# LDeakin/VkVolume

Measured on AMD Instinct MI355X. Metric: Mray/s, higher is better.
Workload: dtype f32

## Files before the change

### vkvolume_amd/csrc/raymarch.hip

```cpp
#include <algorithm>
#include <cmath>
#include <cstdio>
#include <cstdlib>
#include <cstring>
#include <mutex>
#include <new>
#include <vector>

#include "raymarch_inst.hpp"
#include "launchers.hpp"

constexpr int kCostBins = 1024;

__device__ __forceinline__ void tile_order_from_cost(uint32_t *__restrict__ cost, uint32_t *__restrict__ order_out, uint32_t count)
{
	__shared__ uint32_t s_bin[kCostBins];
	constexpr int       kPerThread = 40;
	for (int b = threadIdx.x; b < kCostBins; b += blockDim.x)
		s_bin[b] = 0;
	__syncthreads();
	for (uint32_t base = 0; base < count; base += 256u * kPerThread)
	{
		uint32_t c[kPerThread];
#pragma unroll
// ... 248 lines not shown
{
	const uint32_t tiles_x = (iw + tw - 1) / tw, tiles_y = (ih + th - 1) / th;
	*out = VkvTileRect{0u, 0u, tiles_x, tiles_y};
	double    b[4];
	const int kind = screen_bound(rc->camera_pos_tex, rg->dir00, rg->ddx, rg->ddy, rc->plane_tex, b);
	if (kind == kScreenBoundNone)
		return;
	if (kind == kScreenBoundEmpty || b[0] >= (double) iw || b[2] >= (double) ih)
	{
		*out = VkvTileRect{0u, 0u, 1u, 1u};
		return;
	}
	const uint32_t x0 = b[0] <= 0.0 ? 0u : (uint32_t) b[0], y0 = b[2] <= 0.0 ? 0u : (uint32_t) b[2];
	const uint32_t x1 = b[1] >= (double) (iw - 1) ? iw - 1 : (uint32_t) b[1], y1 = b[3] >= (double) (ih - 1) ? ih - 1 : (uint32_t) b[3];
	const uint32_t q = align > 1 ? align : 1u;
	uint32_t       tx0 = (x0 / tw) / q * q, ty0 = (y0 / th) / q * q;
	uint32_t       tx1 = std::min(tiles_x, (x1 / tw + q) / q * q), ty1 = std::min(tiles_y, (y1 / th + q) / q * q);
	*out = VkvTileRect{tx0, ty0, tx1 - tx0, ty1 - ty0};
}

int fill_render_args(vkv_ctx *ctx, const VkvRenderParams *P, const float *alpha_lut, RayMarchArgs &a, hipStream_t s, const VkvTuning &T, bool setup, bool batch)
{
	for (int i = 0; i < 3; ++i)
	{
		a.dir00[i] = P->ray_gen.dir00[i], a.ddx[i] = P->ray_gen.ddx[i], a.ddy[i] = P->ray_gen.ddy[i];
		a.cam[i]        = P->ray_cast.camera_pos_tex[i];
		a.block_size[i] = P->ray_cast.block_size[i];
	}
	for (int i = 0; i < 4; ++i)
		a.plane_tex[i] = P->ray_cast.plane_tex[i];
	for (int i = 0; i < 16; ++i)
		a.model[i] = P->camera.model[i], a.view[i] = P->camera.camera_view[i], a.proj[i] = P->camera.camera_proj[i],
		a.view_proj_inv[i] = P->camera.camera_view_proj_inv[i], a.model_inv[i] = P->camera.model_inv[i];
	a.sampling_factor = P->transfer_function.sampling_factor;
	a.grad_modifier   = P->transfer_function.grad_magnitude_modifier;
	a.W = (int) P->volume_extent.width, a.H = (int) P->volume_extent.height, a.D = (int) P->volume_extent.depth;
	a.mw = (int) P->map_extent.width, a.mh = (int) P->map_extent.height, a.md = (int) P->map_extent.depth;
	a.vol = P->d_volume, a.grad = P->d_gradient, a.tf = P->d_transfer_function;
	a.packed  = static_cast<const uint8_t *>(P->d_packed_volume);
	a.tf_bits = P->d_transfer_function_bits;
	{
		const PackedDims pd = packed_dims(a.W, a.H, a.D);
		a.pmx = pd.mx, a.pmy = pd.my;
	}
	for (int i = 0; i < 8; ++i)
		a.maps[i] = P->d_distance_maps[i];
	a.out_color = P->d_out_color, a.out_rgba8 = P->d_out_rgba8, a.out_counts = P->d_out_counts, a.out_depth = P->d_out_depth;
	a.in_depth         = P->d_in_depth;
	a.depth_attachment = P->options.depth_attachment != 0, a.blend = P->blend_over_target != 0;
	a.img_w = P->image_width, a.img_h = P->image_height;
	a.tile_w = P->tiles.tile_width, a.tile_h = P->tiles.tile_height;
	a.tile_first = P->tiles.tile_first, a.tile_stride = P->tiles.tile_stride, a.tile_count = P->tiles.tile_count, a.compact = P->tiles.compact;
	a.fill_rgba8_rows = (a.out_rgba8 && !a.out_color && !a.out_counts && !a.out_depth && !a.blend && (a.img_w & 3u) == 0 && (((uintptr_t) a.out_rgba8) & 15u) == 0) ? 1u : 0u;
	bool whole_schedule;
	{
		const VkvTileRect &r = P->tiles.rect;
		const uint32_t     full_x = (a.img_w + a.tile_w - 1) / a.tile_w, full_y = (a.img_h + a.tile_h - 1) / a.tile_h;
		bool               whole  = r.w == 0 || r.h == 0;
		a.fill_tiles = 0, a.img_tiles_x = full_x, a.rect_tx0 = a.rect_ty0 = a.rect_th = 0;
		if (!whole && P->tiles.fill_outside)
		{
			if (!batch || T.scheduler == 1 || T.batch_mode == 1 || (uint64_t) full_x * full_y - (uint64_t) r.w * r.h > (uint64_t) kFillPerTile * r.w * r.h)
				whole = true, a.tile_count = full_x * full_y;
			else
				a.fill_tiles = full_x * full_y - r.w * r.h, a.rect_tx0 = r.x0, a.rect_ty0 = r.y0, a.rect_th = r.h;
		}
// ... 126 lines not shown

	const bool ert  = P->options.early_ray_termination != 0;
	const int  grad = !P->transfer_function.use_gradient ? 0 : (P->use_precomputed_gradient ? 1 : 2);
	const bool sort = sched == (int) kSchedLean && ert && apply_feedback(ctx, a, s);
	int        rc2 = launch_single(ctx, P->options.skipping_type, ert, sched, T, grad, a, s);
	if (rc2 == VKV_OK && sort)
	{
		hipLaunchKernelGGL(k_tile_order_from_cost, dim3(1), dim3(256), 0, s, a.tile_cost, a.order_out, a.tile_count);
		rc2 = check_launch(ctx, "render (start order)");
	}
	return rc2;
}

int prepare_render(vkv_ctx *ctx, const VkvRenderParams *P, uint32_t n, hipStream_t s)
{
	const VkvTuning T = tuning_of(ctx);
	float           lut[256] = {};
	for (uint32_t i = 0; i < n; ++i)
	{
		RayMarchArgs a;
		int rc = fill_render_args(ctx, &P[i], lut, a, s, T, true, false);
		if (rc == VKV_OK && P[i].tiles.fill_outside)
			rc = fill_render_args(ctx, &P[i], lut, a, s, T, true, true);
		if (rc != VKV_OK)
			return rc;
		load_render_code(P[i].options.skipping_type, P[i].options.early_ray_termination != 0);
	}
	load_feedback_code();
	if (!stream_scratch(ctx, s, true).p)
		return VKV_E_UNSUPPORTED;
	return VKV_OK;
}

int launch_render_batch(vkv_ctx *ctx, const VkvRenderParams *P, uint32_t n, const float *alpha_luts, hipStream_t s)
{
	static_assert(kMaxBatch * sizeof(RayMarchArgs) <= kScratchBytes - kBatchArgsOffset, "batch argument blocks must fit the stream scratch");
	static_assert(kPullHeadsBytes + kMaxBatch * sizeof(RayMarchArgs) <= kCaptureSlotBytes, "a captured launch's upload must fit its pinned slot");
	static_assert(kPullHeadsBytes + kMaxBatch * sizeof(RayMarchArgs) <= kUploadSlotBytes, "a launch's upload must fit a slot of the block's pinned ring");
	const VkvTuning     T = tuning_of(ctx);
	const StreamScratch scratch = stream_scratch(ctx, s);
	if (!scratch.p)
		return VKV_E_UNSUPPORTED;
	hipStreamCaptureStatus capture = hipStreamCaptureStatusNone;
	const bool             capturing = hipStreamIsCapturing(s, &capture) == hipSuccess && capture == hipStreamCaptureStatusActive;
	const size_t          upload_bytes = kPullHeadsBytes + n * sizeof(RayMarchArgs);
	vkv_ctx::UploadSlot * ring_slot = nullptr;
	for (uint32_t k = 0; k < vkv_ctx::kUploadRing && !capturing && !ring_slot; ++k)
	{
		vkv_ctx::UploadSlot &u = scratch.block->upload[(scratch.block->upload_next + k) % vkv_ctx::kUploadRing];
		if (!u.pinned)
			continue;
		if (u.pending && hipEventQuery(u.done) == hipSuccess)
			u.pending = false;
		if (!u.pending)
		{
			ring_slot                  = &u;
			scratch.block->upload_next = (scratch.block->upload_next + k + 1) % vkv_ctx::kUploadRing;
		}
	}
	(void) hipGetLastError();
	std::vector<uint8_t> pageable;
	if (!ring_slot)
		pageable.resize(upload_bytes);
	uint8_t *const upload = ring_slot ? ring_slot->pinned : pageable.data();
	std::memset(upload, 0, upload_bytes);
	RayMarchArgs *const host = reinterpret_cast<RayMarchArgs *>(upload + kPullHeadsBytes);
	for (uint32_t i = 0; i < n; ++i)
	{
		const int rc = fill_render_args(ctx, &P[i], alpha_luts + (size_t) i * 256, host[i], s, T, false, true);
		if (rc != VKV_OK)
			return rc;
		if (!host[i].packed)
			return set_error(ctx, VKV_E_INVALID_ARGUMENT, "render_batch: frame %u has no packed sampling image (d_packed_volume)", i);
		if (host[i].blocks_per_tile != host[0].blocks_per_tile)
			return set_error(ctx, VKV_E_INVALID_ARGUMENT, "render_batch: frame %u has a different tile size than frame 0", i);
		if (ctx->d_debug_orders && i < ctx->debug_order_frames && ctx->debug_order_count == host[i].tile_count)
			host[i].tile_order = ctx->d_debug_orders + (size_t) i * ctx->debug_order_count;
	}
	uint32_t max_tiles = 0, ref = 0;
	bool     same_count = true;
	for (uint32_t i = n; i-- > 0;)
	{
		max_tiles = std::max(max_tiles, host[i].nblocks ? host[i].tile_count : 0u);
		if (host[i].nblocks)
			ref = i;
	}
	if (max_tiles == 0)
		return VKV_OK;
	for (uint32_t i = 0; i < n; ++i)
		same_count = same_count && host[i].nblocks != 0 && host[i].tile_count == max_tiles;
	bool any_sort = false;
	for (uint32_t i = 0; i < n && P[0].options.early_ray_termination != 0; ++i)
		any_sort = apply_feedback(ctx, host[i], s) || any_sort;
	RayMarchArgs *   d_frames = reinterpret_cast<RayMarchArgs *>(scratch.p + kBatchArgsOffset);
	uint32_t *       d_heads  = reinterpret_cast<uint32_t *>(scratch.p + kBatchArgsOffset - kPullHeadsBytes);
	const void *upload_src = upload;
	struct SlotGuard
	{
		vkv_ctx *ctx;
		size_t   index;
		bool     armed;
		~SlotGuard()
		{
			if (!armed)
				return;
			std::lock_guard<std::mutex> lock(ctx->mutex);
			if (index < ctx->capture_slots.size())
				ctx->capture_slots[index].in_use = false, ctx->capture_slots[index].owner = VkvStreamKey{};
		}
	} slot_guard{ctx, 0, false};
// ... 95 lines not shown
```

### vkvolume_amd/csrc/raymarch_core.hpp

```cpp
#pragma once

#include <type_traits>

#include "vkv_device.hpp"

using namespace vkv;

constexpr int kTraceWords = 10;
constexpr uint32_t kFillPerTile = 3;

struct RayMarchArgs
{
	float dir00[3], ddx[3], ddy[3];
	float cam[3];
	float plane_tex[4];
	float block_size[3];
	float model[16], view[16], proj[16];
	float view_proj_inv[16], model_inv[16];
	float sampling_factor, grad_modifier;
	int W, H, D, mw, mh, md;
	const uint8_t * vol, *grad, *tf;
	const uint8_t * packed;
	int             pmx, pmy;
	const uint32_t *tf_bits;
	const uint8_t * maps[8];
	float *         out_color;
	uint8_t *       out_rgba8;
	uint32_t *      out_counts;
	float *         out_depth;
	const float *   in_depth;
	uint32_t        depth_attachment, blend;
	uint32_t        img_w, img_h, tile_w, tile_h, tiles_x, tile_first, tile_stride, tile_count, compact;
	uint32_t        org_x, org_y;
	uint32_t        fill_tiles, img_tiles_x, rect_tx0, rect_ty0, rect_th;
	uint32_t        fill_rgba8_rows;
	uint32_t        blocks_per_tile_x, blocks_per_tile, nblocks;
	int             test;
	unsigned long long *trace;
	int             back;
	uint32_t        clamp_always;
	float           mapf[3], mapb[3];
	uint32_t        wave_pw_log2;
	const uint32_t *addr_lut;
	uint32_t        lut_y, lut_z, lut_words;
	uint32_t        lut_full;
	uint32_t        cull_x0, cull_x1, cull_y0, cull_y1;
	const uint32_t *tile_order;
	uint32_t        order_h;
	uint32_t *      queue_heads;
	uint32_t *      tile_cost;
	uint32_t *      order_out;
	float           alpha_lut[256];
};

struct Ray
{
	float          ex, ey, ez;
	float          sx, sy, sz;
	float          six, siy, siz;
	const uint8_t *dmap;
	int            n_steps, i, i_min;
	int            ulx, uly, ulz;
	uint32_t       ul;
	int            first_hit;
	bool           occupied;
	float          r, g, b, a;
	float          depth;
	uint32_t       n_vol, n_dist, n_empty;
	uint32_t       o;
	bool           fragment;
};

__device__ __forceinline__ float sample_linear(const uint8_t *__restrict__ tex, int W, int H, int D, float px, float py, float pz)
{
	const float cx = __builtin_fmaf(px, (float) W, -0.5f), cy = __builtin_fmaf(py, (float) H, -0.5f), cz = __builtin_fmaf(pz, (float) D, -0.5f);
	const float fx = __builtin_floorf(cx), fy = __builtin_floorf(cy), fz = __builtin_floorf(cz);
	const float wx = cx - fx, wy = cy - fy, wz = cz - fz;
	const int   ix = (int) fx, iy = (int) fy, iz = (int) fz;
	const int   x0 = i_clamp(ix, 0, W - 1), x1 = i_clamp(ix + 1, 0, W - 1);
	const int   y0 = i_clamp(iy, 0, H - 1), y1 = i_clamp(iy + 1, 0, H - 1);
	const int   z0 = i_clamp(iz, 0, D - 1), z1 = i_clamp(iz + 1, 0, D - 1);
	const size_t r00 = ((size_t) z0 * (size_t) H + (size_t) y0) * (size_t) W, r10 = ((size_t) z0 * (size_t) H + (size_t) y1) * (size_t) W;
	const size_t r01 = ((size_t) z1 * (size_t) H + (size_t) y0) * (size_t) W, r11 = ((size_t) z1 * (size_t) H + (size_t) y1) * (size_t) W;
	const float b000 = tex[r00 + x0], b100 = tex[r00 + x1];
	const float b010 = tex[r10 + x0], b110 = tex[r10 + x1];
	const float b001 = tex[r01 + x0], b101 = tex[r01 + x1];
// ... 648 lines not shown
		}
		if (n_idle == 64)
			break;
		if (active)
		{
			if (ray_event<SKIP, ERT, GRAD, PACKED>(A, R, s_alpha, s_unorm, s_bits, tf_bits))
			{
				ray_finish(A, R, true);
				active = false;
			}
		}
	}
}


struct RmLds
{
	union
	{
		struct
		{
			float    alpha[256];
			uint32_t bits[2048];
			float    unorm[256];
		} g;
		struct
		{
			float  ai[258], ag[258];
			float2 pair[256];
		} s;
	};
};

__device__ __forceinline__ bool tf_is_separable(const RayMarchArgs &A)
{
	return A.tf_bits != nullptr && (A.tf_bits[kTfFlagWord] & kTfFlagSeparable) != 0u;
}

__device__ __forceinline__ bool stage_tables_er(const RayMarchArgs &A, RmLds &L, bool sync = true)
{
	const bool sep = tf_is_separable(A);
	typedef const __attribute__((address_space(1))) uint32_t *global_u32_ptr;
	const global_u32_ptr tf_words = (global_u32_ptr) (uintptr_t) A.tf_bits;
	for (int i = threadIdx.x; i < 256; i += blockDim.x)
	{
		const float a = A.alpha_lut[i];
		if (!sep)
			L.g.alpha[i] = a;
		if (sep)
		{
			const float ai = __uint_as_float(tf_words[kTfAiWord + i]), ag = __uint_as_float(tf_words[kTfAgWord + i]);
			L.s.ai[i] = ai, L.s.ag[i] = ag;
			if (i == 255)
				L.s.ai[256] = ai, L.s.ag[256] = ag;
			L.s.pair[i] = i == 0 ? make_float2(0.0f, 0.0f) : make_float2(a, unorm8(i) * a);
		}
		else
			L.g.unorm[i] = unorm8(i);
	}
	if (!sep && A.tf_bits)
		for (int i = threadIdx.x; i < 2048; i += blockDim.x)
			L.g.bits[i] = A.tf_bits[i];
	if (sync)
		__syncthreads();
	return sep;
}
template <int W>
__device__ __forceinline__ bool block_pixel(const RayMarchArgs &A, uint32_t b, uint32_t rb, uint32_t &px, uint32_t &py, uint32_t &o)
{
	constexpr uint32_t G = 64 / W;
	uint32_t           bx, by;
	const uint32_t     wb = rb / G, g = rb % G;
	if (W == 1)
	{
		const uint32_t pwl = A.wave_pw_log2, pprl = 4u - pwl;
		bx = ((wb & ((1u << pprl) - 1u)) << pwl) + (g & ((1u << pwl) - 1u));
		by = ((wb >> pprl) << (6u - pwl)) + (g >> pwl);
	}
	else
	{
		constexpr uint32_t pw = G >= 32 ? 8 : (G >= 8 ? 4 : 2), ph = G / pw, ppr = 16 / pw;
		bx = (wb % ppr) * pw + g % pw, by = (wb / ppr) * ph + g / pw;
	}
	const uint32_t k = b / A.blocks_per_tile, sb = b % A.blocks_per_tile;
	const uint32_t t  = A.tile_first + k * A.tile_stride;
	const uint32_t lx = (sb % A.blocks_per_tile_x) * 16 + bx, ly = (sb / A.blocks_per_tile_x) * 16 + by;
	px = A.org_x + (t % A.tiles_x) * A.tile_w + lx, py = A.org_y + (t / A.tiles_x) * A.tile_h + ly;
	o  = A.compact ? (k * A.tile_h + ly) * A.tile_w + lx : py * A.img_w + px;
	return px < A.img_w && py < A.img_h;
}
__device__ __forceinline__ int med3_i32(int x, int lo, int hi)
// ... 86 lines not shown
		const float c0 = __builtin_fmaf(wy, c10 - c00, c00), c1 = __builtin_fmaf(wy, c11 - c01, c01);
		out_g = __builtin_fmaf(wz, c1 - c0, c0) * kScale;
	}
}
extern __shared__ __align__(16) uint32_t s_lean_lds[];
static_assert(sizeof(RmLds) % 16 == 0, "the address tables behind RmLds are read as 64-bit words");

typedef __attribute__((address_space(3))) RmLds *   lds_rmlds_ptr;
typedef __attribute__((address_space(3))) uint32_t *lds_u32_ptr;

constexpr uintptr_t kLdsBase = 16;
__device__ __forceinline__ RmLds &lean_lds() { return *(RmLds *) (lds_rmlds_ptr) kLdsBase; }

__device__ __forceinline__ void lean_lds_check()
{
	uint32_t base = (uint32_t) reinterpret_cast<uintptr_t>(s_lean_lds);
	asm volatile("" : "+s"(base));
	if (base != 0u)
		__builtin_trap();
}

__device__ __forceinline__ bool wg_any(bool pred)
{
	uint32_t *flags = (uint32_t *) (lds_u32_ptr) kLdsBase;
	const bool mine = __builtin_amdgcn_ballot_w64(pred) != 0ull;
	if ((threadIdx.x & 63u) == 0u)
		flags[threadIdx.x >> 6] = mine ? 1u : 0u;
	__syncthreads();
	const uint32_t nw  = blockDim.x >> 6;
	const uint4    f   = *reinterpret_cast<const uint4 *>(flags);
	const bool     any = (f.x | (nw > 1u ? f.y : 0u) | (nw > 2u ? f.z : 0u) | (nw > 3u ? f.w : 0u)) != 0u;
	__syncthreads();
	return any;
}

#define s_addr_lut ((uint32_t *) (lds_u32_ptr) (kLdsBase + sizeof(RmLds)))
constexpr uint32_t kLutXm = 96;

__device__ __forceinline__ void stage_addr_lut(const RayMarchArgs &A)
{
	for (uint32_t i = threadIdx.x; i < A.lut_z; i += blockDim.x)
		s_addr_lut[i] = A.addr_lut[i];
	const uint64_t base = reinterpret_cast<uint64_t>(A.packed);
	for (uint32_t i = threadIdx.x; 2 * i + A.lut_z < A.lut_words; i += blockDim.x)
	{
		const uint64_t z = (((uint64_t) A.addr_lut[A.lut_z + 2 * i + 1]) << 32 | A.addr_lut[A.lut_z + 2 * i]) + base;
		s_addr_lut[A.lut_z + 2 * i] = (uint32_t) z, s_addr_lut[A.lut_z + 2 * i + 1] = (uint32_t) (z >> 32);
	}
}

template <bool SC = true>
__device__ __forceinline__ const uint8_t *packed_footprint_lut(const RayMarchArgs &A, float px, float py, float pz, float &wx, float &wy, float &wz)
{
	const float cx = __builtin_fmaf(px, (float) A.W, -0.5f), cy = __builtin_fmaf(py, (float) A.H, -0.5f), cz = __builtin_fmaf(pz, (float) A.D, -0.5f);
	const float fx = __builtin_floorf(cx), fy = __builtin_floorf(cy), fz = __builtin_floorf(cz);
	wx = cx - fx, wy = cy - fy, wz = cz - fz;
	const uint32_t tx = (uint32_t) (SC ? clamp0_i32((int) __builtin_fmaf(fx, 4.0f, 4.0f), 4 * (A.W + 1)) : med3_i32((int) __builtin_fmaf(fx, 4.0f, 4.0f), 0, 4 * (A.W + 1)));
	const uint32_t ty = (uint32_t) (SC ? clamp0_i32((int) __builtin_fmaf(fy, 4.0f, 4.0f), 4 * (A.H + 1)) : med3_i32((int) __builtin_fmaf(fy, 4.0f, 4.0f), 0, 4 * (A.H + 1)));
	const uint32_t tz = (uint32_t) (SC ? clamp0_i32((int) __builtin_fmaf(fz, 4.0f, 4.0f), 4 * (A.D + 1)) : med3_i32((int) __builtin_fmaf(fz, 4.0f, 4.0f), 0, 4 * (A.D + 1)));
	const char *   lut = reinterpret_cast<const char *>(s_addr_lut);
	const uint32_t xi = *reinterpret_cast<const uint32_t *>(lut + (tx & 124u)), xm = *reinterpret_cast<const uint32_t *>(lut + 4u * kLutXm + ((tx >> 5) & ~3u));
	const uint32_t yi = *reinterpret_cast<const uint32_t *>(lut + 128u + (ty & 124u)), ym = *reinterpret_cast<const uint32_t *>(lut + 4u * A.lut_y + ((ty >> 5) & ~3u));
	const uint32_t zi = *reinterpret_cast<const uint32_t *>(lut + 256u + (tz & 124u));
	const uint64_t zm = *reinterpret_cast<const uint64_t *>(lut + 4u * A.lut_z + ((tz >> 4) & ~7u));
	return reinterpret_cast<const uint8_t *>(zm + (((xi + xm) + (yi + ym)) + zi));
}
// ... 28 lines not shown
	uint32_t nvec;
};

__device__ __forceinline__ FullLutCopy full_lut_issue(const RayMarchArgs &A)
{
	typedef const __attribute__((address_space(1))) lut_v4u *global_v4u_ptr;
	FullLutCopy          c;
	const global_v4u_ptr g = (global_v4u_ptr) (uintptr_t) (A.addr_lut + A.lut_full);
	c.nvec                 = ((uint32_t) (A.W + 2 + A.H + 2 + A.D + 2) + 3u) >> 2;
#pragma unroll
	for (uint32_t k = 0; k < kFullCopyRounds; ++k)
		c.r[k] = g[min(threadIdx.x + k * blockDim.x, c.nvec - 1u)];
	return c;
}

__device__ __forceinline__ void full_lut_commit(const RayMarchArgs &A, const FullLutCopy &c, RmLds &L)
{
	static_assert(sizeof(((RmLds *) nullptr)->s) == kFullLutWord * 4, "full tables start behind the separable TF tables");
	typedef const __attribute__((address_space(1))) lut_v4u *global_v4u_ptr;
	lut_v4u *dst = reinterpret_cast<lut_v4u *>(full_lut_base(L));
#pragma unroll
	for (uint32_t k = 0; k < kFullCopyRounds; ++k)
		if (threadIdx.x + k * blockDim.x < c.nvec)
			dst[threadIdx.x + k * blockDim.x] = c.r[k];
	const global_v4u_ptr g = (global_v4u_ptr) (uintptr_t) (A.addr_lut + A.lut_full);
	for (uint32_t i = threadIdx.x + kFullCopyRounds * blockDim.x; i < c.nvec; i += blockDim.x)
		dst[i] = g[i];
}

__device__ __forceinline__ void stage_full_lut(const RayMarchArgs &A, RmLds &L)
{
	const FullLutCopy c = full_lut_issue(A);
	full_lut_commit(A, c, L);
}

struct FullLutConsts
{
	float          w, h, d, oy, oz;
	const uint8_t *base;
};

template <bool SCALAR = false>
__device__ __forceinline__ FullLutConsts full_lut_consts(const RayMarchArgs &A)
{
	FullLutConsts c;
	c.w = (float) A.W, c.h = (float) A.H, c.d = (float) A.D;
	c.base = A.packed;
	c.oy = (float) (4 * (A.W + 2) + 4);
	c.oz = (float) (4 * (A.W + 2 + A.H + 2) + 4);
	if (SCALAR)
		c.w = uniform_f32(c.w), c.h = uniform_f32(c.h), c.d = uniform_f32(c.d), c.oy = uniform_f32(c.oy), c.oz = uniform_f32(c.oz);
	else
		asm volatile("" : "+v"(c.w), "+v"(c.h), "+v"(c.d), "+v"(c.oy), "+v"(c.oz));
	return c;
}

template <bool FREE = false>
__device__ __forceinline__ const uint8_t *packed_footprint_full(const FullLutConsts &C, const RmLds &L, float px, float py, float pz, float &wx, float &wy, float &wz)
{
	const float cx = __builtin_fmaf(px, C.w, -0.5f), cy = __builtin_fmaf(py, C.h, -0.5f), cz = __builtin_fmaf(pz, C.d, -0.5f);
	const float fx = __builtin_floorf(cx), fy = __builtin_floorf(cy), fz = __builtin_floorf(cz);
	wx = cx - fx, wy = cy - fy, wz = cz - fz;
	const int   tx = (int) __builtin_fmaf(FREE ? fx : __builtin_amdgcn_fmed3f(fx, -1.0f, C.w), 4.0f, 4.0f);
	const int   ty = (int) __builtin_fmaf(FREE ? fy : __builtin_amdgcn_fmed3f(fy, -1.0f, C.h), 4.0f, C.oy);
	const int   tz = (int) __builtin_fmaf(FREE ? fz : __builtin_amdgcn_fmed3f(fz, -1.0f, C.d), 4.0f, C.oz);
	const char *   lut = reinterpret_cast<const char *>(full_lut_base(L));
// ... 370 lines not shown
		R.a = R.a > 0.99f ? 1.0f : R.a;
	if (SEP)
		R.r = grey, R.g = grey, R.b = grey;
}

__device__ __forceinline__ uint32_t start_entry(const RayMarchArgs &A, uint32_t r)
{
	const int w = (int) A.tiles_x, h = (int) A.order_h, rings = (min(w, h) + 1) >> 1;
	auto      inner = [&](int j) { return (w - 2 * j > 0 && h - 2 * j > 0) ? (uint32_t) ((w - 2 * j) * (h - 2 * j)) : 0u; };
	const float d = (float) (w - h);
	int         j = (int) (((float) (w + h) - __builtin_sqrtf(d * d + 4.0f * (float) r)) * 0.25f);
	j             = max(0, min(j, rings - 1));
#pragma unroll
	for (int it = 0; it < 2; ++it)
	{
		if (j + 1 < rings && inner(j + 1) > r)
			++j;
		if (j > 0 && inner(j) <= r)
			--j;
	}
	const int wj = w - 2 * j, hj = h - 2 * j;
	int       q = (int) (r - inner(j + 1)), tx, ty;
	if (hj == 1 || q < wj)
		tx = j + q, ty = j;
	else if ((q -= wj) < hj - 1)
		tx = j + wj - 1, ty = j + 1 + q;
	else if ((q -= hj - 1) < wj - 1)
		tx = j + wj - 2 - q, ty = j + hj - 1;
	else
		q -= wj - 1, tx = j, ty = j + hj - 2 - q;
	return (uint32_t) __builtin_amdgcn_readfirstlane(ty * w + tx);
}

template <int SKIP, bool ERT, int GRAD, bool PACKED, uint32_t LF, int WPB = 4, bool FILL = false>
__device__ __forceinline__ void lean_block(const RayMarchArgs &A, uint32_t bid, RmLds &L)
{
	constexpr uint32_t kParts = 4 / WPB;
	const uint32_t x = bid & 7u, idx = (bid >> 3) / kParts, part = (bid >> 3) % kParts;
	const uint32_t rank = (idx / A.blocks_per_tile) * 8u + x, sb = idx % A.blocks_per_tile;
	if (rank >= A.tile_count)
		return;
	const uint32_t k = A.tile_order ? A.tile_order[rank] : (A.order_h ? start_entry(A, rank) : rank);
	if (k >= A.tile_count)
		return;
	const uint32_t lane = threadIdx.x & 63u, wave = threadIdx.x >> 6;
	uint32_t       px, py, o;
	const uint32_t rb = (part * WPB + wave) * 64u + lane;
	if (FILL && A.fill_tiles != 0u)
	{
#pragma unroll
		for (uint32_t it = 0; it < kFillPerTile; ++it)
		{
			const uint32_t j = k + it * A.tile_count;
			if (j >= A.fill_tiles)
				break;
			const uint32_t top = A.rect_ty0 * A.img_tiles_x, per_row = A.img_tiles_x - A.tiles_x, mid = A.rect_th * per_row;
			uint32_t       tx, ty;
			if (j < top)
				ty = j / A.img_tiles_x, tx = j % A.img_tiles_x;
			else if (j - top < mid)
			{
				const uint32_t q = j - top, c = q % per_row;
				ty = A.rect_ty0 + q / per_row, tx = c < A.rect_tx0 ? c : c + A.tiles_x;
			}
			else
			{
				const uint32_t q = j - top - mid;
				ty = A.rect_ty0 + A.rect_th + q / A.img_tiles_x, tx = q % A.img_tiles_x;
			}
			const uint32_t bx0 = tx * A.tile_w + (sb % A.blocks_per_tile_x) * 16u, by0 = ty * A.tile_h + (sb / A.blocks_per_tile_x) * 16u;
			if (A.fill_rgba8_rows != 0u && bx0 + 16u <= A.img_w)
			{
				if (rb < 64u && by0 + (rb >> 2) < A.img_h)
				{
					typedef uint32_t v4u __attribute__((ext_vector_type(4)));
					const v4u zero = {0u, 0u, 0u, 0u};
					__builtin_nontemporal_store(zero, reinterpret_cast<v4u *>(A.out_rgba8 + ((size_t) (by0 + (rb >> 2)) * A.img_w + bx0 + (rb & 3u) * 4u) * 4u));
				}
			}
			else
			{
				const uint32_t fx = bx0 + (rb & 15u), fy = by0 + (rb >> 4);
				if (fx < A.img_w && fy < A.img_h)
				{
					Ray F;
					ray_clear(F);
					F.o = fy * A.img_w + fx;
					ray_finish(A, F, false);
				}
			}
		}
	}
	const bool     inside = block_pixel<1>(A, k * A.blocks_per_tile + sb, rb, px, py, o);
	Ray R;
	R.o = o;
	const unsigned long long t_start = A.trace ? __builtin_amdgcn_s_memrealtime() : 0ull;
	const unsigned long long c_start = A.trace ? __builtin_amdgcn_s_memtime() : 0ull;
	bool marched = false;
	if (inside)
	{
		if (px >= A.cull_x0 && px <= A.cull_x1 && py >= A.cull_y0 && py <= A.cull_y1)
			marched = ray_setup<SKIP>(A, px, py, R);
		else
			ray_clear(R);
	}
	uint32_t  iter  = 0;
	LeanStamp stamp = {};
	if (wg_any(marched))
	{
		bool sep;
		if ((LF & kLeanLut) != 0 && (LF & kLeanFull) != 0 && PACKED && GRAD != 2 && tf_is_separable(A))
		{
			const FullLutCopy c = full_lut_issue(A);
			sep                 = stage_tables_er(A, L, false);
			full_lut_commit(A, c, L);
			__syncthreads();
		}
		else
		{
			if ((LF & kLeanLut) != 0 && PACKED && GRAD != 2)
				stage_addr_lut(A);
			sep = stage_tables_er(A, L);
		}
		if (marched)
		{
			if (sep)
			{
				constexpr bool kSafe = (LF & kLeanSafe) != 0 && (LF & kLeanFull) != 0 && PACKED && GRAD != 2 && SKIP != VKV_SKIP_NONE && (LF & kLeanStamp) == 0;
				if constexpr (kSafe)
				{
					if (lean_free_wave(A, R))
						lean_march<SKIP, ERT, GRAD, PACKED, true, LF, true>(A, R, L, iter, stamp);
					else
						lean_march<SKIP, ERT, GRAD, PACKED, true, LF>(A, R, L, iter, stamp);
				}
				else
					lean_march<SKIP, ERT, GRAD, PACKED, true, LF>(A, R, L, iter, stamp);
			}
			else
				lean_march<SKIP, ERT, GRAD, PACKED, false, LF>(A, R, L, iter, stamp);
		}
	}
	if (A.tile_cost)
	{
// ... 20 lines not shown
			unsigned long long *rec = A.trace + ((size_t) blockIdx.x * WPB + wave) * kTraceWords;
			rec[4] = ((unsigned long long) stamp.cnt[0] << 32) | stamp.sum[0], rec[5] = ((unsigned long long) stamp.cnt[1] << 32) | stamp.sum[1];
			rec[8] = ((unsigned long long) stamp.cnt[2] << 32) | stamp.sum[2];
		}
		else if ((LF & kLeanStamp) == 0 && lane == (uint32_t) __builtin_ctzll(__ballot(1)))
		{
			unsigned long long *rec = A.trace + ((size_t) blockIdx.x * WPB + wave) * kTraceWords;
			rec[4] = 0, rec[5] = 0, rec[8] = 0;
		}
		if (lane == (uint32_t) __builtin_ctzll(__ballot(1)))
		{
			unsigned long long *rec = A.trace + ((size_t) blockIdx.x * WPB + wave) * kTraceWords;
			rec[0] = t_start, rec[1] = t_end, rec[2] = it, rec[3] = ((unsigned long long) __builtin_amdgcn_s_getreg((3 << 11) | 20) << 32) | (k * A.blocks_per_tile + sb);
			rec[6] = c_start, rec[7] = __builtin_amdgcn_s_memtime(), rec[9] = clamped_max;
		}
	}
}

#if defined(__HIP_DEVICE_COMPILE__) && !defined(VKV_LAB_PACKED_FP32)
#define VKV_NO_PACKED_FP32 __attribute__((target("no-packed-fp32-ops")))
#else
#define VKV_NO_PACKED_FP32
#endif

template <int SKIP, bool ERT, int GRAD, bool PACKED, uint32_t LF>
__global__ void __launch_bounds__(256) k_raymarch_lean(const RayMarchArgs A)
{
	lean_lds_check();
	RmLds &L = lean_lds();
	lean_block<SKIP, ERT, GRAD, PACKED, LF>(A, blockIdx.x, L);
}

template <int SKIP, bool ERT, int GRAD, uint32_t LF>
__global__ void __launch_bounds__(256) VKV_NO_PACKED_FP32 __attribute__((amdgpu_waves_per_eu((GRAD == 2 || SKIP == VKV_SKIP_NONE || (LF & kLeanLut) == 0) ? 1 : 8))) k_raymarch_lean_batch(const RayMarchArgs *__restrict__ frames, uint32_t n, uint32_t groups_per_frame)
{
	lean_lds_check();
	RmLds &        L = lean_lds();
	const uint32_t g = blockIdx.x >> 3;
	const uint32_t f = groups_per_frame == 0 ? g % n : g / groups_per_frame, gi = groups_per_frame == 0 ? g / n : g % groups_per_frame;
	constexpr uint32_t kLfBatch = (SKIP == VKV_SKIP_ANISOTROPIC_DISTANCE && (LF & kLeanNoCounts) == 0) ? (LF & ~kLeanSafe) : LF;
	lean_block<SKIP, ERT, GRAD, true, kLfBatch, 4, true>(frames[f], (gi << 3) | (blockIdx.x & 7u), L);
}

template <int SKIP, bool ERT, int GRAD, uint32_t LF, bool SEP>
__device__ __forceinline__ void pull_units(const RayMarchArgs *__restrict__ frames, uint32_t n, uint32_t *__restrict__ heads, const RmLds &L)
{
	const RayMarchArgs &A0   = frames[0];
	const uint32_t      lane = threadIdx.x & 63u;
	const uint32_t      upt  = A0.blocks_per_tile * 4u;
	uint32_t            q = blockIdx.x & 7u, open_queues = 0xffu;
	while (open_queues != 0u)
	{
		if (((open_queues >> q) & 1u) == 0u)
		{
			q = (q + 1u) & 7u;
			continue;
		}
		uint32_t v = 0;
		if (lane == 0)
			v = atomicAdd(&heads[q * vkv::kPullHeadStride], 1u);
		v = __builtin_amdgcn_readfirstlane(v);
		const uint32_t tiles_q = A0.tile_count > q ? (A0.tile_count - q + 7u) >> 3 : 0u;
		if (v >= tiles_q * upt * n)
		{
			open_queues &= ~(1u << q);
			q = (q + 1u) & 7u;
			continue;
		}
		const uint32_t      w = v % upt, f = (v / upt) % n, rank = (v / (upt * n)) * 8u + q;
		const RayMarchArgs &A = frames[f];
		const uint32_t      k = A.tile_order ? A.tile_order[rank] : rank;
		if (k >= A.tile_count)
			continue;
		uint32_t            px, py, o;
// ... 78 lines not shown
```

### vkvolume_amd/csrc/raymarch_inst.hpp

```cpp
#pragma once

#include "raymarch_core.hpp"

namespace vkv
{

enum Scheduler
{
	kSchedLean       = 0,
	kSchedPersistent = 1
};

constexpr uint32_t kLfPlain  = 0;
constexpr uint32_t kLfLut    = kLeanLut;
#ifdef VKV_LEAN_NO_ASYNC
constexpr uint32_t kLfFull   = kLeanLut | kLeanFull | kLeanSafe;
#else
constexpr uint32_t kLfFull   = kLeanLut | kLeanFull | kLeanSafe | kLeanAsync;
#endif
constexpr uint32_t kLfFullNc = kLfFull | kLeanNoCounts;
constexpr uint32_t kLfLutNc  = kLfLut | kLeanNoCounts;

struct LeanChoice
{
// ... 57 lines not shown
						hipLaunchKernelGGL((k_raymarch_lean<SKIP, ERT, GRAD, PACKED, kLfLutNc>), dim3(grid), dim3(256), c.lds, s, a);
				}
			}
			else if (c.kind == 2)
				hipLaunchKernelGGL((k_raymarch_lean<SKIP, ERT, GRAD, PACKED, kLfFull>), dim3(grid), dim3(256), c.lds, s, a);
			else if (c.kind == 1)
				hipLaunchKernelGGL((k_raymarch_lean<SKIP, ERT, GRAD, PACKED, kLfLut>), dim3(grid), dim3(256), c.lds, s, a);
			launched = c.kind != 0;
		}
		if (!launched)
			hipLaunchKernelGGL((k_raymarch_lean<SKIP, ERT, GRAD, PACKED, kLfPlain>), dim3(grid), dim3(256), lean_lds_bytes(0, 0, a.W, a.H, a.D), s, a);
	}
	return check_launch(ctx, "render");
}

template <int SKIP, bool ERT>
int RayMarchLaunchers<SKIP, ERT>::single(vkv_ctx *ctx, int sched, const VkvTuning &T, int grad, RayMarchArgs &a, hipStream_t s)
{
	if (a.packed)
		return grad == 0 ? launch_one<SKIP, ERT, 0, true>(ctx, sched, T, a, s) : (grad == 1 ? launch_one<SKIP, ERT, 1, true>(ctx, sched, T, a, s) : launch_one<SKIP, ERT, 2, true>(ctx, sched, T, a, s));
	return grad == 0 ? launch_one<SKIP, ERT, 0, false>(ctx, sched, T, a, s) : (grad == 1 ? launch_one<SKIP, ERT, 1, false>(ctx, sched, T, a, s) : launch_one<SKIP, ERT, 2, false>(ctx, sched, T, a, s));
}

template <int SKIP, bool ERT>
void RayMarchLaunchers<SKIP, ERT>::load()
{
	hipFuncAttributes at;
	(void) hipFuncGetAttributes(&at, reinterpret_cast<const void *>(&k_raymarch_lean<SKIP, ERT, 0, true, kLfPlain>));
}

template <int SKIP, bool ERT, int GRAD>
static void launch_batch_kind(LeanChoice c, bool no_counts, const RayMarchArgs *d_frames, uint32_t n, uint32_t grid, uint32_t gpf, hipStream_t s)
{
	if constexpr (GRAD != 2)
	{
		if constexpr (SKIP != VKV_SKIP_NONE && ERT && GRAD == 1)
		{
			if (c.kind != 0 && no_counts)
			{
				if (c.kind == 2)
					hipLaunchKernelGGL((k_raymarch_lean_batch<SKIP, ERT, GRAD, kLfFullNc>), dim3(grid), dim3(256), c.lds, s, d_frames, n, gpf);
				else
					hipLaunchKernelGGL((k_raymarch_lean_batch<SKIP, ERT, GRAD, kLfLutNc>), dim3(grid), dim3(256), c.lds, s, d_frames, n, gpf);
				return;
			}
		}
		if (c.kind == 2)
			hipLaunchKernelGGL((k_raymarch_lean_batch<SKIP, ERT, GRAD, kLfFull>), dim3(grid), dim3(256), c.lds, s, d_frames, n, gpf);
		else if (c.kind == 1)
			hipLaunchKernelGGL((k_raymarch_lean_batch<SKIP, ERT, GRAD, kLfLut>), dim3(grid), dim3(256), c.lds, s, d_frames, n, gpf);
		if (c.kind != 0)
			return;
	}
	hipLaunchKernelGGL((k_raymarch_lean_batch<SKIP, ERT, GRAD, kLfPlain>), dim3(grid), dim3(256), lean_lds_bytes(0, 0, 0, 0, 0), s, d_frames, n, gpf);
}

template <int SKIP, bool ERT>
void RayMarchLaunchers<SKIP, ERT>::batch(int grad, const RayMarchArgs *d_frames, uint32_t n, uint32_t grid, uint32_t gpf, LeanChoice c, bool no_counts, hipStream_t s)
{
	if (grad == 0)
		launch_batch_kind<SKIP, ERT, 0>(c, no_counts, d_frames, n, grid, gpf, s);
	else if (grad == 1)
		launch_batch_kind<SKIP, ERT, 1>(c, no_counts, d_frames, n, grid, gpf, s);
	else
		launch_batch_kind<SKIP, ERT, 2>(c, no_counts, d_frames, n, grid, gpf, s);
}

template <int SKIP, bool ERT, int GRAD, uint32_t LF>
static uint32_t launch_pull_one(vkv_ctx *ctx, const RayMarchArgs *d_frames, uint32_t n, uint32_t *d_heads, size_t lds, uint64_t units, hipStream_t s)
{
	const uint64_t resident = (uint64_t) 8 * (uint64_t) (ctx->cu_count > 1 ? ctx->cu_count : 1);
	const uint64_t want     = resident < (units + 3) / 4 ? resident : (units + 3) / 4;
	const uint32_t grid     = (uint32_t) (want < 8 ? 8 : want);
	hipLaunchKernelGGL((k_raymarch_lean_pull<SKIP, ERT, GRAD, LF>), dim3(grid), dim3(256), lds, s, d_frames, n, d_heads);
	return grid;
}

template <int SKIP, bool ERT, int GRAD>
static uint32_t launch_pull_kind(vkv_ctx *ctx, LeanChoice c, const RayMarchArgs *d_frames, uint32_t n, uint32_t *d_heads, uint64_t units, hipStream_t s)
{
	if constexpr (GRAD != 2)
	{
		if (c.kind == 2)
			return launch_pull_one<SKIP, ERT, GRAD, kLfFull>(ctx, d_frames, n, d_heads, c.lds, units, s);
		if (c.kind == 1)
			return launch_pull_one<SKIP, ERT, GRAD, kLfLut>(ctx, d_frames, n, d_heads, c.lds, units, s);
	}
// ... 25 lines not shown
```

### vkvolume_amd/csrc/vkv_device.hpp

```cpp
#pragma once

#include <hip/hip_runtime.h>
#include <stdint.h>

#include <map>
#include <memory>
#include <mutex>
#include <thread>
#include <unordered_map>
#include <vector>

#include "../../include/vkvolume_amd.h"

namespace vkv
{

__device__ __forceinline__ float g_min(float x, float y) { return (y < x) ? y : x; }
__device__ __forceinline__ float g_max(float x, float y) { return (x < y) ? y : x; }
__device__ __forceinline__ float g_clamp(float x, float lo, float hi) { return g_min(g_max(x, lo), hi); }
__device__ __forceinline__ float g_step(float edge, float x) { return (x < edge) ? 0.0f : 1.0f; }
__device__ __forceinline__ float g_sign(float x) { return (x > 0.0f) ? 1.0f : ((x < 0.0f) ? -1.0f : 0.0f); }
__device__ __forceinline__ int   i_clamp(int x, int lo, int hi) { return min(max(x, lo), hi); }

constexpr float kInv255 = 1.0f / 255.0f;
// ... 206 lines not shown
		uint32_t *  d_cost, *d_order;
		bool        has_cost;
		uint32_t    frames;
		uint32_t    measured_at = 0;
		uint32_t    period = 8;
		uint32_t    used = 0;
		float       view_dir[3] = {0, 0, 0}, view_pos[3] = {0, 0, 0};
		float       prev_dir[3] = {0, 0, 0}, prev_pos[3] = {0, 0, 0};
		bool        has_prev = false;
	};
	std::vector<TileFeedback *> feedback;
};

namespace vkv
{
int  set_error(vkv_ctx *ctx, int code, const char *fmt, ...);
int  check_launch(vkv_ctx *ctx, const char *what);
int  check_box(vkv_ctx *ctx, const char *what, VkvExtent3D extent, const VkvBox *box);
VkvStreamKey stream_key(hipStream_t stream);
struct StreamScratch
{
	uint8_t *                    p = nullptr;
	std::unique_lock<std::mutex> lock;
	vkv_ctx::ScratchBlock *      block = nullptr;
};
StreamScratch stream_scratch(vkv_ctx *ctx, hipStream_t stream, bool setup = false);
const uint32_t *packed_addr_lut(vkv_ctx *ctx, int W, int H, int D, uint32_t *lut_y, uint32_t *lut_z, uint32_t *words, uint32_t *full, hipStream_t stream, bool setup = false);
const uint32_t *tile_start_order(vkv_ctx *ctx, uint32_t img_w, uint32_t img_h, uint32_t tile_w, uint32_t tile_h, uint32_t first, uint32_t stride, uint32_t count,
                                 hipStream_t stream, bool setup = false);
VkvTuning tuning_of(vkv_ctx *ctx);
constexpr size_t kScratchBytes     = 128 * 1024;
constexpr size_t kScratchReserve   = 16;
constexpr uint32_t kCaptureSlots   = 32;
constexpr size_t   kUploadSlotBytes = 64 * 1024;
constexpr size_t   kAlphaLuts = 8;
constexpr size_t   kCaptureSlotBytes = 96 * 1024;
constexpr uint32_t kMaxDynamicLds  = 64 * 1024 - 1024;
constexpr size_t kTfBitsOffset     = 0;
constexpr size_t kQueueHeadsOffset = 8192 + 64;
constexpr size_t kTfRangesOffset   = 16 * 1024;
constexpr size_t kPullHeadsBytes   = 2048;
constexpr uint32_t kPullHeadStride = 64;
constexpr size_t kBatchArgsOffset  = 32 * 1024 + kPullHeadsBytes;
constexpr uint32_t kMaxBatch       = VKV_MAX_BATCH;
static_assert(kTfRangesOffset >= kQueueHeadsOffset + 32 && kTfRangesOffset + 4 * 2048 * 8 <= kScratchBytes, "the range table must fit the scratch block");

struct DeviceGuard
{
	int  prev = -1;
	bool switched = false;
	explicit DeviceGuard(int device)
	{
		if (hipGetDevice(&prev) == hipSuccess && prev != device)
			switched = hipSetDevice(device) == hipSuccess;
	}
	~DeviceGuard()
	{
		if (switched)
			(void) hipSetDevice(prev);
	}
	DeviceGuard(const DeviceGuard &) = delete;
	DeviceGuard &operator=(const DeviceGuard &) = delete;
};
}
```

Measured before the change: 22350.

## Precompute pair LUT images on host and stage LDS tables via global_load_lds

Builds deduplicated per-frame alpha/premultiplied pair tables on the host, uploads them with the batch arguments, and has the lean batch kernel copy them, along with the address LUT and separable TF tables, straight into LDS using global_load_lds DMA instructions issued early, before the march setup. The aim is to take the per-workgroup table staging (ALU work plus register round-trips) off the critical path and overlap it with ray setup. It also swaps unorm8 computation for a constant table and splits wg_any into a publish/any pair so one barrier covers both the flag and the DMA wait. In exchange it adds inline asm that writes M0, enlarges the upload slots, and issues the copies unconditionally for tiles that may not march.

```diff
diff --git a/vkvolume_amd/csrc/raymarch.hip b/vkvolume_amd/csrc/raymarch.hip
--- a/vkvolume_amd/csrc/raymarch.hip
+++ b/vkvolume_amd/csrc/raymarch.hip
@@ -304,6 +304,7 @@
 	for (int i = 0; i < 16; ++i)
 		a.model[i] = P->camera.model[i], a.view[i] = P->camera.camera_view[i], a.proj[i] = P->camera.camera_proj[i],
 		a.view_proj_inv[i] = P->camera.camera_view_proj_inv[i], a.model_inv[i] = P->camera.model_inv[i];
+	a.pair_off        = 0;
 	a.sampling_factor = P->transfer_function.sampling_factor;
 	a.grad_modifier   = P->transfer_function.grad_magnitude_modifier;
 	a.W = (int) P->volume_extent.width, a.H = (int) P->volume_extent.height, a.D = (int) P->volume_extent.depth;
@@ -496,18 +497,32 @@
 	return VKV_OK;
 }
 
+void build_pair_image(const float *alpha_lut, float *image)
+{
+	image[0] = image[1] = 0.0f;
+	for (uint32_t b = 1; b < 256; ++b)
+	{
+		const float a = alpha_lut[b], u = (float) b / 255.0f;
+		image[2 * b] = a, image[2 * b + 1] = u * a;
+	}
+}
+
 int launch_render_batch(vkv_ctx *ctx, const VkvRenderParams *P, uint32_t n, const float *alpha_luts, hipStream_t s)
 {
 	static_assert(kMaxBatch * sizeof(RayMarchArgs) <= kScratchBytes - kBatchArgsOffset, "batch argument blocks must fit the stream scratch");
-	static_assert(kPullHeadsBytes + kMaxBatch * sizeof(RayMarchArgs) <= kCaptureSlotBytes, "a captured launch's upload must fit its pinned slot");
-	static_assert(kPullHeadsBytes + kMaxBatch * sizeof(RayMarchArgs) <= kUploadSlotBytes, "a launch's upload must fit a slot of the block's pinned ring");
+	constexpr size_t kMaxUploadBytes = ((kPullHeadsBytes + kMaxBatch * sizeof(RayMarchArgs) + 15) & ~(size_t) 15) + (size_t) kPairImages * kPairImageBytes;
+	static_assert(kBatchArgsOffset - kPullHeadsBytes + kMaxUploadBytes <= kScratchBytes, "argument blocks and pair images must fit the stream scratch");
+	static_assert(kMaxUploadBytes <= kCaptureSlotBytes, "a captured launch's upload must fit its pinned slot");
+	static_assert(kMaxUploadBytes <= kUploadSlotBytes, "a launch's upload must fit a slot of the block's pinned ring");
+	static_assert(kPullHeadsBytes % 16 == 0 && kBatchArgsOffset % 16 == 0, "the pair images are read in 16-byte pieces");
 	const VkvTuning     T = tuning_of(ctx);
 	const StreamScratch scratch = stream_scratch(ctx, s);
 	if (!scratch.p)
 		return VKV_E_UNSUPPORTED;
 	hipStreamCaptureStatus capture = hipStreamCaptureStatusNone;
 	const bool             capturing = hipStreamIsCapturing(s, &capture) == hipSuccess && capture == hipStreamCaptureStatusActive;
-	const size_t          upload_bytes = kPullHeadsBytes + n * sizeof(RayMarchArgs);
+	const size_t          args_bytes = kPullHeadsBytes + n * sizeof(RayMarchArgs), pair_base = (args_bytes + 15) & ~(size_t) 15;
+	size_t                upload_bytes = pair_base;
 	vkv_ctx::UploadSlot * ring_slot = nullptr;
 	for (uint32_t k = 0; k < vkv_ctx::kUploadRing && !capturing && !ring_slot; ++k)
 	{
@@ -525,9 +540,9 @@
 	(void) hipGetLastError();
 	std::vector<uint8_t> pageable;
 	if (!ring_slot)
-		pageable.resize(upload_bytes);
+		pageable.resize(pair_base + (size_t) kPairImages * kPairImageBytes);
 	uint8_t *const upload = ring_slot ? ring_slot->pinned : pageable.data();
-	std::memset(upload, 0, upload_bytes);
+	std::memset(upload, 0, pair_base);
 	RayMarchArgs *const host = reinterpret_cast<RayMarchArgs *>(upload + kPullHeadsBytes);
 	for (uint32_t i = 0; i < n; ++i)
 	{
@@ -540,6 +555,27 @@
 			return set_error(ctx, VKV_E_INVALID_ARGUMENT, "render_batch: frame %u has a different tile size than frame 0", i);
 		if (ctx->d_debug_orders && i < ctx->debug_order_frames && ctx->debug_order_count == host[i].tile_count)
 			host[i].tile_order = ctx->d_debug_orders + (size_t) i * ctx->debug_order_count;
+	}
+	{
+		uint32_t n_images = 0, image_of[kMaxBatch];
+		for (uint32_t i = 0; i < n; ++i)
+		{
+			image_of[i] = ~0u;
+			if (host[i].nblocks == 0)
+				continue;
+			for (uint32_t j = 0; j < i && image_of[i] == ~0u; ++j)
+				if (image_of[j] != ~0u && std::memcmp(host[j].alpha_lut, host[i].alpha_lut, sizeof(host[i].alpha_lut)) == 0)
+					image_of[i] = image_of[j];
+			if (image_of[i] == ~0u && n_images < kPairImages)
+			{
+				float *img = reinterpret_cast<float *>(upload + pair_base + (size_t) n_images * kPairImageBytes);
+				build_pair_image(host[i].alpha_lut, img);
+				image_of[i] = n_images++;
+			}
+			if (image_of[i] != ~0u)
+				host[i].pair_off = (uint32_t) (pair_base + (size_t) image_of[i] * kPairImageBytes);
+		}
+		upload_bytes = pair_base + (size_t) n_images * kPairImageBytes;
 	}
 	uint32_t max_tiles = 0, ref = 0;
 	bool     same_count = true;
diff --git a/vkvolume_amd/csrc/raymarch_core.hpp b/vkvolume_amd/csrc/raymarch_core.hpp
--- a/vkvolume_amd/csrc/raymarch_core.hpp
+++ b/vkvolume_amd/csrc/raymarch_core.hpp
@@ -47,11 +47,16 @@
 	uint32_t        cull_x0, cull_x1, cull_y0, cull_y1;
 	const uint32_t *tile_order;
 	uint32_t        order_h;
+	uint32_t        pair_off;
 	uint32_t *      queue_heads;
 	uint32_t *      tile_cost;
 	uint32_t *      order_out;
 	float           alpha_lut[256];
 };
+static_assert(offsetof(RayMarchArgs, queue_heads) == offsetof(RayMarchArgs, order_h) + 8, "pair_off sits in what was padding: the block does not grow");
+static_assert(sizeof(RayMarchArgs) % 8 == 0, "argument blocks follow each other in one upload");
+constexpr uint32_t kPairImageBytes = 256 * 8;
+constexpr uint32_t kPairImages     = 8;
 
 struct Ray
 {
@@ -766,6 +771,17 @@
 	};
 };
 
+struct Unorm8Table
+{
+	float v[256];
+	constexpr Unorm8Table() : v()
+	{
+		for (int i = 0; i < 256; ++i)
+			v[i] = (float) i / 255.0f;
+	}
+};
+static __constant__ const Unorm8Table kUnorm8Table{};
+
 __device__ __forceinline__ bool tf_is_separable(const RayMarchArgs &A)
 {
 	return A.tf_bits != nullptr && (A.tf_bits[kTfFlagWord] & kTfFlagSeparable) != 0u;
@@ -787,10 +803,10 @@
 			L.s.ai[i] = ai, L.s.ag[i] = ag;
 			if (i == 255)
 				L.s.ai[256] = ai, L.s.ag[256] = ag;
-			L.s.pair[i] = i == 0 ? make_float2(0.0f, 0.0f) : make_float2(a, unorm8(i) * a);
+			L.s.pair[i] = i == 0 ? make_float2(0.0f, 0.0f) : make_float2(a, kUnorm8Table.v[i] * a);
 		}
 		else
-			L.g.unorm[i] = unorm8(i);
+			L.g.unorm[i] = kUnorm8Table.v[i];
 	}
 	if (!sep && A.tf_bits)
 		for (int i = threadIdx.x; i < 2048; i += blockDim.x)
@@ -943,6 +959,20 @@
 	const bool     any = (f.x | (nw > 1u ? f.y : 0u) | (nw > 2u ? f.z : 0u) | (nw > 3u ? f.w : 0u)) != 0u;
 	__syncthreads();
 	return any;
+}
+
+__device__ __forceinline__ void wg_flag_publish(bool pred)
+{
+	static_assert(kLdsBase >= 16, "one flag word per wave of a workgroup of up to four");
+	const bool mine = __builtin_amdgcn_ballot_w64(pred) != 0ull;
+	if ((threadIdx.x & 63u) == 0u)
+		s_lean_lds[threadIdx.x >> 6] = mine ? 1u : 0u;
+}
+__device__ __forceinline__ bool wg_flag_any()
+{
+	const uint32_t nw = blockDim.x >> 6;
+	const uint4    f  = *reinterpret_cast<const uint4 *>(s_lean_lds);
+	return (f.x | (nw > 1u ? f.y : 0u) | (nw > 2u ? f.z : 0u) | (nw > 3u ? f.w : 0u)) != 0u;
 }
 
 #define s_addr_lut ((uint32_t *) (lds_u32_ptr) (kLdsBase + sizeof(RmLds)))
@@ -1037,6 +1067,66 @@
 {
 	const FullLutCopy c = full_lut_issue(A);
 	full_lut_commit(A, c, L);
+}
+
+__device__ __forceinline__ void glds16(uintptr_t src, uint32_t lds_byte_address)
+{
+	uint32_t keep;
+	asm volatile("s_mov_b32 %0, m0\n\ts_mov_b32 m0, %2\n\ts_nop 0\n\tglobal_load_lds_dwordx4 %1, off\n\ts_mov_b32 m0, %0" : "=&s"(keep) : "v"(src), "s"(lds_byte_address));
+}
+__device__ __forceinline__ void glds4(uintptr_t src, uint32_t lds_byte_address)
+{
+	uint32_t keep;
+	asm volatile("s_mov_b32 %0, m0\n\ts_mov_b32 m0, %2\n\ts_nop 0\n\tglobal_load_lds_dword %1, off\n\ts_mov_b32 m0, %0" : "=&s"(keep) : "v"(src), "s"(lds_byte_address));
+}
+__device__ __forceinline__ void lean_image_wait() { asm volatile("s_waitcnt vmcnt(0)" ::: "memory"); }
+
+template <bool PAIR>
+__device__ __forceinline__ void lean_image_issue(const RayMarchArgs &A, const uint8_t *upload)
+{
+	static_assert(offsetof(RmLds, s.pair) % 16 == 0 && kLdsBase % 16 == 0, "pair[] is copied in 16-byte pieces");
+	const uint32_t t  = threadIdx.x, nt = blockDim.x;
+	const uint32_t wf = (uint32_t) __builtin_amdgcn_readfirstlane((int) (t & ~63u));
+	{
+		const uintptr_t g    = (uintptr_t) (A.addr_lut + A.lut_full);
+		const uint32_t  nvec = ((uint32_t) (A.W + 2 + A.H + 2 + A.D + 2) + 3u) >> 2;
+		for (uint32_t first = 0; first < nvec; first += nt)
+			if (first + t < nvec)
+				glds16(g + (size_t) (first + t) * 16u, (uint32_t) kLdsBase + kFullLutWord * 4u + (first + wf) * 16u);
+	}
+	{
+		const uintptr_t tf = (uintptr_t) A.tf_bits;
+		for (uint32_t first = 0; first < 256u; first += nt)
+		{
+			const uint32_t i = first + t;
+			if (i < 256u)
+			{
+				glds4(tf + (size_t) (kTfAiWord + i) * 4u, (uint32_t) (kLdsBase + offsetof(RmLds, s.ai)) + (first + wf) * 4u);
+				glds4(tf + (size_t) (kTfAgWord + i) * 4u, (uint32_t) (kLdsBase + offsetof(RmLds, s.ag)) + (first + wf) * 4u);
+			}
+			if (i == 255u)
+			{
+				glds4(tf + (size_t) (kTfAiWord + i) * 4u, (uint32_t) (kLdsBase + offsetof(RmLds, s.ai)) + (first + wf + 1u) * 4u);
+				glds4(tf + (size_t) (kTfAgWord + i) * 4u, (uint32_t) (kLdsBase + offsetof(RmLds, s.ag)) + (first + wf + 1u) * 4u);
+			}
+		}
+	}
+	if (PAIR && A.pair_off != 0u)
+	{
+		const uintptr_t p = (uintptr_t) upload + A.pair_off;
+		for (uint32_t first = 0; first < kPairImageBytes / 16u; first += nt)
+			if (first + t < kPairImageBytes / 16u)
+				glds16(p + (size_t) (first + t) * 16u, (uint32_t) (kLdsBase + offsetof(RmLds, s.pair)) + (first + wf) * 16u);
+	}
+}
+
+__device__ __forceinline__ void stage_pair(const RayMarchArgs &A, RmLds &L)
+{
+	for (uint32_t i = threadIdx.x; i < 256u; i += blockDim.x)
+	{
+		const float a = A.alpha_lut[i];
+		L.s.pair[i]   = i == 0u ? make_float2(0.0f, 0.0f) : make_float2(a, kUnorm8Table.v[i] * a);
+	}
 }
 
 struct FullLutConsts
@@ -1473,8 +1563,8 @@
 	return (uint32_t) __builtin_amdgcn_readfirstlane(ty * w + tx);
 }
 
-template <int SKIP, bool ERT, int GRAD, bool PACKED, uint32_t LF, int WPB = 4, bool FILL = false>
-__device__ __forceinline__ void lean_block(const RayMarchArgs &A, uint32_t bid, RmLds &L)
+template <int SKIP, bool ERT, int GRAD, bool PACKED, uint32_t LF, int WPB = 4, bool FILL = false, bool PAIR = false>
+__device__ __forceinline__ void lean_block(const RayMarchArgs &A, uint32_t bid, RmLds &L, const uint8_t *upload = nullptr)
 {
 	constexpr uint32_t kParts = 4 / WPB;
 	const uint32_t x = bid & 7u, idx = (bid >> 3) / kParts, part = (bid >> 3) % kParts;
@@ -1487,6 +1577,19 @@
 	const uint32_t lane = threadIdx.x & 63u, wave = threadIdx.x >> 6;
 	uint32_t       px, py, o;
 	const uint32_t rb = (part * WPB + wave) * 64u + lane;
+	constexpr bool kImage = PAIR && (LF & kLeanLut) != 0 && (LF & kLeanFull) != 0 && PACKED && GRAD != 2;
+	bool           image  = false;
+	if constexpr (kImage)
+	{
+		if (tf_is_separable(A))
+		{
+			image = true;
+			const uint32_t t0  = A.tile_first + k * A.tile_stride;
+			const uint32_t bx0 = A.org_x + (t0 % A.tiles_x) * A.tile_w + (sb % A.blocks_per_tile_x) * 16u, by0 = A.org_y + (t0 / A.tiles_x) * A.tile_h + (sb / A.blocks_per_tile_x) * 16u;
+			if (bx0 <= A.cull_x1 && bx0 + 15u >= A.cull_x0 && by0 <= A.cull_y1 && by0 + 15u >= A.cull_y0)
+				lean_image_issue<PAIR>(A, upload);
+		}
+	}
 	if (FILL && A.fill_tiles != 0u)
 	{
 #pragma unroll
@@ -1547,10 +1650,23 @@
 	}
 	uint32_t  iter  = 0;
 	LeanStamp stamp = {};
-	if (wg_any(marched))
+	wg_flag_publish(marched);
+	if constexpr (kImage)
+		lean_image_wait();
+	__syncthreads();
+	if (wg_flag_any())
 	{
 		bool sep;
-		if ((LF & kLeanLut) != 0 && (LF & kLeanFull) != 0 && PACKED && GRAD != 2 && tf_is_separable(A))
+		if (image)
+		{
+			sep = true;
+			if (A.pair_off == 0u)
+			{
+				stage_pair(A, L);
+				__syncthreads();
+			}
+		}
+		else if ((LF & kLeanLut) != 0 && (LF & kLeanFull) != 0 && PACKED && GRAD != 2 && tf_is_separable(A))
 		{
 			const FullLutCopy c = full_lut_issue(A);
 			sep                 = stage_tables_er(A, L, false);
@@ -1637,14 +1753,14 @@
 }
 
 template <int SKIP, bool ERT, int GRAD, uint32_t LF>
-__global__ void __launch_bounds__(256) VKV_NO_PACKED_FP32 __attribute__((amdgpu_waves_per_eu((GRAD == 2 || SKIP == VKV_SKIP_NONE || (LF & kLeanLut) == 0) ? 1 : 8))) k_raymarch_lean_batch(const RayMarchArgs *__restrict__ frames, uint32_t n, uint32_t groups_per_frame)
+__global__ void __launch_bounds__(256) VKV_NO_PACKED_FP32 __attribute__((amdgpu_waves_per_eu((GRAD == 2 || SKIP == VKV_SKIP_NONE || (LF & kLeanLut) == 0) ? 1 : 8))) k_raymarch_lean_batch(const RayMarchArgs *__restrict__ frames, uint32_t n, uint32_t groups_per_frame, const uint8_t *__restrict__ upload)
 {
 	lean_lds_check();
 	RmLds &        L = lean_lds();
 	const uint32_t g = blockIdx.x >> 3;
 	const uint32_t f = groups_per_frame == 0 ? g % n : g / groups_per_frame, gi = groups_per_frame == 0 ? g / n : g % groups_per_frame;
 	constexpr uint32_t kLfBatch = (SKIP == VKV_SKIP_ANISOTROPIC_DISTANCE && (LF & kLeanNoCounts) == 0) ? (LF & ~kLeanSafe) : LF;
-	lean_block<SKIP, ERT, GRAD, true, kLfBatch, 4, true>(frames[f], (gi << 3) | (blockIdx.x & 7u), L);
+	lean_block<SKIP, ERT, GRAD, true, kLfBatch, 4, true, true>(frames[f], (gi << 3) | (blockIdx.x & 7u), L, upload);
 }
 
 template <int SKIP, bool ERT, int GRAD, uint32_t LF, bool SEP>
diff --git a/vkvolume_amd/csrc/raymarch_inst.hpp b/vkvolume_amd/csrc/raymarch_inst.hpp
--- a/vkvolume_amd/csrc/raymarch_inst.hpp
+++ b/vkvolume_amd/csrc/raymarch_inst.hpp
@@ -113,6 +113,7 @@
 template <int SKIP, bool ERT, int GRAD>
 static void launch_batch_kind(LeanChoice c, bool no_counts, const RayMarchArgs *d_frames, uint32_t n, uint32_t grid, uint32_t gpf, hipStream_t s)
 {
+	const uint8_t *upload = reinterpret_cast<const uint8_t *>(d_frames) - kPullHeadsBytes;
 	if constexpr (GRAD != 2)
 	{
 		if constexpr (SKIP != VKV_SKIP_NONE && ERT && GRAD == 1)
@@ -120,20 +121,20 @@
 			if (c.kind != 0 && no_counts)
 			{
 				if (c.kind == 2)
-					hipLaunchKernelGGL((k_raymarch_lean_batch<SKIP, ERT, GRAD, kLfFullNc>), dim3(grid), dim3(256), c.lds, s, d_frames, n, gpf);
+					hipLaunchKernelGGL((k_raymarch_lean_batch<SKIP, ERT, GRAD, kLfFullNc>), dim3(grid), dim3(256), c.lds, s, d_frames, n, gpf, upload);
 				else
-					hipLaunchKernelGGL((k_raymarch_lean_batch<SKIP, ERT, GRAD, kLfLutNc>), dim3(grid), dim3(256), c.lds, s, d_frames, n, gpf);
+					hipLaunchKernelGGL((k_raymarch_lean_batch<SKIP, ERT, GRAD, kLfLutNc>), dim3(grid), dim3(256), c.lds, s, d_frames, n, gpf, upload);
 				return;
 			}
 		}
 		if (c.kind == 2)
-			hipLaunchKernelGGL((k_raymarch_lean_batch<SKIP, ERT, GRAD, kLfFull>), dim3(grid), dim3(256), c.lds, s, d_frames, n, gpf);
+			hipLaunchKernelGGL((k_raymarch_lean_batch<SKIP, ERT, GRAD, kLfFull>), dim3(grid), dim3(256), c.lds, s, d_frames, n, gpf, upload);
 		else if (c.kind == 1)
-			hipLaunchKernelGGL((k_raymarch_lean_batch<SKIP, ERT, GRAD, kLfLut>), dim3(grid), dim3(256), c.lds, s, d_frames, n, gpf);
+			hipLaunchKernelGGL((k_raymarch_lean_batch<SKIP, ERT, GRAD, kLfLut>), dim3(grid), dim3(256), c.lds, s, d_frames, n, gpf, upload);
 		if (c.kind != 0)
 			return;
 	}
-	hipLaunchKernelGGL((k_raymarch_lean_batch<SKIP, ERT, GRAD, kLfPlain>), dim3(grid), dim3(256), lean_lds_bytes(0, 0, 0, 0, 0), s, d_frames, n, gpf);
+	hipLaunchKernelGGL((k_raymarch_lean_batch<SKIP, ERT, GRAD, kLfPlain>), dim3(grid), dim3(256), lean_lds_bytes(0, 0, 0, 0, 0), s, d_frames, n, gpf, upload);
 }
 
 template <int SKIP, bool ERT>
diff --git a/vkvolume_amd/csrc/vkv_device.hpp b/vkvolume_amd/csrc/vkv_device.hpp
--- a/vkvolume_amd/csrc/vkv_device.hpp
+++ b/vkvolume_amd/csrc/vkv_device.hpp
@@ -262,7 +262,7 @@
 constexpr size_t kScratchBytes     = 128 * 1024;
 constexpr size_t kScratchReserve   = 16;
 constexpr uint32_t kCaptureSlots   = 32;
-constexpr size_t   kUploadSlotBytes = 64 * 1024;
+constexpr size_t   kUploadSlotBytes = 80 * 1024;
 constexpr size_t   kAlphaLuts = 8;
 constexpr size_t   kCaptureSlotBytes = 96 * 1024;
 constexpr uint32_t kMaxDynamicLds  = 64 * 1024 - 1024;
```

Measured after the change: 22030. -1.4%, worse.
